# yzqin/s4g-release

Measured on AMD Instinct MI355X. Metric: scenes/sec (25.6k-pt clouds) end-to-end grasp inference, higher is better.
Workload: dtype f32 (f16x2 split)

## Files before the change

include/s4g_ops.h:

```cpp
#ifndef S4G_OPS_H_
#define S4G_OPS_H_

#include <stddef.h>
#include <stdint.h>

#ifdef __cplusplus
extern "C" {
#endif

#define S4G_ABI_VERSION 14


#define S4G_OK 0
#define S4G_EINVAL (-1)
#define S4G_EWORKSPACE (-2)
#define S4G_EUNSUPPORTED (-3)

#define S4G_FLAG_FMAD 1

typedef void *s4g_stream_t;

#define S4G_OP_FPS 1
#define S4G_OP_BALL_QUERY 2
#define S4G_OP_THREE_NN 3
// ... 135 lines not shown
} s4g_gemm_desc_t;

int s4g_mlp_gemm_f32(const s4g_gemm_desc_t *desc, s4g_stream_t stream);

typedef struct s4g_heads_desc {
  int32_t precision, P, N, ldx;
  int32_t C, H0, H1, H2, H3;
  const float *X;
  const void *W_frag[5];
  const float *bias[5];
  const float *w_inv_scale[5];
  float *out[4];
  int32_t channels[4];
  int32_t sigmoid_head;
  const float *a_amax;
  float a_amax_floor;
  int32_t rows_per_scene;
  const void *pre_W_frag[2];
  const float *pre_bias[2];
  const float *pre_w_inv_scale[2];
  const int32_t *pre_nidx;
  const float *pre_nw;
  const float *pre_sparse;
  const float *pre_dense;
  const float *pre_lbias;
  const float *pre_a_amax2;
  int32_t pre_N2;
  int64_t out_batch_stride;
  int32_t head_mask;
} s4g_heads_desc_t;

int s4g_heads_chain_f32(const s4g_heads_desc_t *desc, s4g_stream_t stream);

int s4g_amax_per_scene_f32(const float *x, int64_t B, int64_t n_per_scene, float *out_slots, s4g_stream_t stream);

int s4g_gemm_chain_supported(int loader, int epilogue, int C, int Kpad16);

int s4g_ball_query_i32(const float *xyz_b3n, const float *ctr_b3m, int64_t B,
                       int64_t N, int64_t M, float radius, int64_t K,
                       int32_t *idx_bmk, int32_t *cnt_bm, void *ws,
                       size_t ws_bytes, int flags, s4g_stream_t stream);
int s4g_three_nn_weights_i32(const float *q_b3n1, const float *k_b3n2, int64_t B,
                             int64_t N1, int64_t N2, float eps, int32_t *idx_bn3,
                             float *w_bn3, void *ws, size_t ws_bytes, int flags,
                             s4g_stream_t stream);
size_t s4g_three_nn_grid_workspace_bytes(int64_t B, int64_t N1, int64_t N2);
size_t s4g_three_nn_grid_header_offset(int64_t B, int64_t N2);
int s4g_three_nn_weights_grid_i32(const float *q_b3n1, const float *k_b3n2, int64_t B,
                                  int64_t N1, int64_t N2, float eps, float cell,
                                  int32_t *idx_bn3, float *w_bn3, void *ws,
                                  size_t ws_bytes, int flags, s4g_stream_t stream);

int s4g_three_nn_grid_f32(const float *q_b3n1, const float *k_b3n2, int64_t B, int64_t N1,
                          int64_t N2, float cell, int64_t *idx_bn3, float *d2_bn3, void *ws,
                          size_t ws_bytes, int flags, s4g_stream_t stream);

int s4g_query_group_f32(const float *xyz_b3n, const float *ctr_b3m, int64_t B,
                        int64_t N, int64_t M, float radius, int64_t K,
                        int64_t *idx_bmk, int64_t *cnt_bm, float *grouped_b3mk,
                        void *ws, size_t ws_bytes, int flags, s4g_stream_t stream);

int s4g_group_rel_xyz_i32(const float *xyz_b3n, const float *ctr_b3m, const int32_t *idx_bmk,
                          int64_t B, int64_t N, int64_t M, int64_t K, float *rel_pk4,
                          s4g_stream_t stream);

int s4g_group_rel_xyz_unique_i32(const float *xyz_b3n, const float *ctr_b3m, const int32_t *idx_bmk,
// ... 185 lines not shown
```

s4g_release_amd/_cabi.py:

```python
import ctypes
import os

_HERE = os.path.dirname(os.path.abspath(__file__))
LIB_PATH = os.environ.get("S4G_HIP_LIB") or os.path.join(_HERE, "libs4g_hip.so")

S4G_ABI_VERSION = 14
S4G_EINVAL = -1
S4G_EWORKSPACE = -2
S4G_EUNSUPPORTED = -3
S4G_FLAG_FMAD = 1
S4G_OP_FPS, S4G_OP_BALL_QUERY, S4G_OP_THREE_NN = 1, 2, 3

_vp = ctypes.c_void_p
_i64 = ctypes.c_int64
_sz = ctypes.c_size_t
_int = ctypes.c_int
_f32 = ctypes.c_float

_i32 = ctypes.c_int32


class GemmDesc(ctypes.Structure):
    _fields_ = [
        ("loader", _i32), ("epilogue", _i32), ("groups", _i32), ("relu", _i32),
# ... 3 lines not shown
        ("gidx", _vp), ("feat", _vp), ("xyz", _vp), ("ctr", _vp),
        ("Cf", _i32), ("N", _i32), ("M", _i32), ("K", _i32),
        ("nidx", _vp), ("nw", _vp), ("sparse", _vp), ("dense", _vp),
        ("C2", _i32), ("C1", _i32), ("N2", _i32), ("N1", _i32),
        ("out", _vp), ("ldc", _i32), ("c_coff", _i32), ("c_gcol", _i32),
        ("cf_ptr", _vp * 4), ("cf_start", _i32 * 5), ("cf_sigmoid_from", _i32), ("cf_N", _i32),
        ("precision", _i32), ("Kpad16", _i32), ("W_bf16x3", _vp), ("mlp1_w", _vp),
        ("W_f16x2", _vp), ("w_inv_scale", _vp), ("a_amax", _vp), ("a_amax2", _vp),
        ("a_amax_floor", _f32), ("out_amax", _vp), ("W_f16x2_frag", _vp),
        ("W2_f16x2_frag", _vp), ("w2_inv_scale", _vp), ("bias2", _vp), ("Cout2", _i32), ("relu2", _i32),
        ("W3_f16x2_frag", _vp), ("w3_inv_scale", _vp), ("bias3", _vp), ("Cout3", _i32), ("relu3", _i32),
        ("loader_bias", _vp), ("rows_per_scene", _i32), ("rel_xyz4", _vp), ("seg4", _vp), ("seg_rows", _vp),
        ("out2", _vp), ("ldc2", _i32), ("split_n", _i32), ("out_amax2", _vp),
        ("a_L", _i32),
    ]


class HeadsDesc(ctypes.Structure):
    _fields_ = [
        ("precision", _i32), ("P", _i32), ("N", _i32), ("ldx", _i32),
        ("C", _i32), ("H0", _i32), ("H1", _i32), ("H2", _i32), ("H3", _i32),
        ("X", _vp), ("W_frag", _vp * 5), ("bias", _vp * 5), ("w_inv_scale", _vp * 5),
        ("out", _vp * 4), ("channels", _i32 * 4), ("sigmoid_head", _i32),
        ("a_amax", _vp), ("a_amax_floor", _f32), ("rows_per_scene", _i32),
        ("pre_W_frag", _vp * 2), ("pre_bias", _vp * 2), ("pre_w_inv_scale", _vp * 2),
        ("pre_nidx", _vp), ("pre_nw", _vp), ("pre_sparse", _vp), ("pre_dense", _vp),
        ("pre_lbias", _vp), ("pre_a_amax2", _vp), ("pre_N2", _i32), ("out_batch_stride", _i64), ("head_mask", _i32),
    ]


SIGNATURES = {
    "s4g_mlp_gemm_f32": (_int, [ctypes.POINTER(GemmDesc), _vp]),
    "s4g_heads_chain_f32": (_int, [ctypes.POINTER(HeadsDesc), _vp]),
    "s4g_ball_query_i32": (_int, [_vp, _vp, _i64, _i64, _i64, _f32, _i64, _vp, _vp, _vp, _sz,
                                  _int, _vp]),
    "s4g_three_nn_weights_i32": (_int, [_vp, _vp, _i64, _i64, _i64, _f32, _vp, _vp, _vp, _sz,
                                        _int, _vp]),
    "s4g_three_nn_grid_workspace_bytes": (_sz, [_i64, _i64, _i64]),
    "s4g_three_nn_grid_header_offset": (_sz, [_i64, _i64]),
    "s4g_three_nn_weights_grid_i32": (_int, [_vp, _vp, _i64, _i64, _i64, _f32, _f32, _vp, _vp, _vp,
                                             _sz, _int, _vp]),
    "s4g_three_nn_grid_f32": (_int, [_vp, _vp, _i64, _i64, _i64, _f32, _vp, _vp, _vp, _sz, _int, _vp]),
    "s4g_group_points_xyz_f32": (_int, [_vp, _vp, _i64, _i64, _i64, _i64, _vp, _vp, _sz, _vp]),
    "s4g_gemm_chain_supported": (_int, [_int, _int, _int, _int]),
    "s4g_amax_per_scene_f32": (_int, [_vp, _i64, _i64, _vp, _vp]),
    "s4g_interp_add_cl_f32": (_int, [_vp, _vp, _vp, _vp, _vp, _i64, _i64, _i64, _i64, _int, _vp, _vp, _vp]),
    "s4g_group_points_ws_f32": (_int, [_vp, _vp, _i64, _i64, _i64, _i64, _i64, _vp, _vp, _sz, _vp]),
    "s4g_three_interpolate_ws_f32": (_int, [_vp, _vp, _vp, _i64, _i64, _i64, _i64, _vp, _vp, _sz, _int, _vp]),
    "s4g_fps_gather_i32": (_int, [_vp, _i64, _i64, _i64, _vp, _vp, _vp, _sz, _int, _vp]),
    "s4g_fps_prepass_f32": (_int, [_vp, _i64, _i64, _i64, _vp, _vp, _vp]),
    "s4g_fps_gather_ex_i32": (_int, [_vp, _i64, _i64, _i64, _vp, _vp, _vp, _vp, _vp, _sz, _int, _vp]),
    "s4g_fps_prefix_check_f32": (_int, [_vp, _vp, _i64, _i64, _i64, _vp, _int, _vp]),
    "s4g_build_variants": (_int, []),
    "s4g_test_knobs_enabled": (_int, []),
    "s4g_fps_f64": (_int, [_vp, _i64, _i64, _i64, _vp, _vp, _sz, _int, _vp]),
    "s4g_ball_query_f64": (_int, [_vp, _vp, _i64, _i64, _i64, _f32, _i64, _vp, _vp, _int, _vp]),
    "s4g_three_nn_f64": (_int, [_vp, _vp, _i64, _i64, _i64, _vp, _vp, _int, _vp]),
    "s4g_group_points_f64": (_int, [_vp, _vp, _i64, _i64, _i64, _i64, _i64, _vp, _vp]),
    "s4g_group_points_backward_f64": (_int, [_vp, _vp, _i64, _i64, _i64, _i64, _i64, _vp, _vp]),
    "s4g_three_interpolate_f64": (_int, [_vp, _vp, _vp, _i64, _i64, _i64, _i64, _vp, _int, _vp]),
    "s4g_three_interpolate_backward_f64": (_int, [_vp, _vp, _vp, _i64, _i64, _i64, _i64, _vp, _vp]),
    "s4g_scatter_det_workspace_bytes": (_sz, [_i64, _i64, _i64]),
    "s4g_scatter_det_workspace_bytes_c": (_sz, [_i64, _i64, _i64, _i64, _int]),
    "s4g_group_points_backward_det_f32": (_int, [_vp, _vp, _i64, _i64, _i64, _i64, _i64, _vp, _vp, _sz, _vp]),
    "s4g_three_interpolate_backward_det_f32": (_int, [_vp, _vp, _vp, _i64, _i64, _i64, _i64, _vp, _vp, _sz, _vp]),
    "s4g_group_rel_xyz_i32": (_int, [_vp, _vp, _vp, _i64, _i64, _i64, _i64, _vp, _vp]),
# ... 127 lines not shown
```

s4g_release_amd/csrc/mlp_heads.hip:

```cpp
#include <stdlib.h>

#include "mlp_common.h"

#ifndef S4G_HEADS_ABLATE
#define S4G_HEADS_ABLATE 0
#endif

namespace s4g {

__device__ __forceinline__ void heads_keep_alive(const f32x16& v) { asm volatile("" ::"v"(v)); }

struct HeadsParams {
  int P, N;
  const float* X;
  int ldx;
  const uint16_t* W[5];
  const float* bias[5];
  const float* wsc[5];
  float* out[4];
  int ch[4];
  long long obs[4];
  int head_mask;
  int sigmoid_head;
  const float* a_amax;
  float a_floor;
  int rps;
  const uint16_t* Wp[2];
  const float* bias_p[2];
  const float* wsc_p[2];
  const int* nidx;
  const float* nw;
  const float* sparse;
  const float* dense;
  const float* lbias;
  const float* a_amax2;
  int N2;
};

template <int PL, int HD_RING, int NRBT, bool PRE>
__global__ __launch_bounds__(512, 2) void mlp_heads_kernel(const HeadsParams p) {
  constexpr int BM = 32 * NRBT, C = 256, NW = 8, astr = C + 8, aplane = BM * astr;
  constexpr int FB = PL * 1024;
  extern __shared__ __attribute__((aligned(16))) float smemf[];
  uint16_t* PA = reinterpret_cast<uint16_t*>(smemf);
  uint16_t* PB = PA + PL * aplane;
  float* scr = reinterpret_cast<float*>(PB + PL * aplane);

  const int t = threadIdx.x;
  const int lane = t & 63;
  const int li = lane & 31, lh = lane >> 5;
  const int wv = __builtin_amdgcn_readfirstlane(t >> 6);
  const int p0 = blockIdx.x * BM;
  const uint32_t wf_lane = (uint32_t)lane * 16u;

  float sa = 1.f, inv_sa = 1.f;
  if constexpr (PL == 2) {
    float amax = p.a_floor;
    if constexpr (PRE) {
      if (p.a_amax) amax += amax_rows(p.a_amax, lane, p0, min(p0 + BM, p.P) - 1, p.rps);
      if (p.a_amax2) amax += amax_rows(p.a_amax2, lane, p0, min(p0 + BM, p.P) - 1, p.rps);
    } else if (p.a_amax) {
      amax = fmaxf(amax, amax_rows(p.a_amax, lane, p0, min(p0 + BM, p.P) - 1, p.rps));
    }
    uint32_t ex = __float_as_uint(amax) >> 23;
    ex = ex < 15u ? 15u : (ex > 240u ? 240u : ex);
    ex = __builtin_amdgcn_readfirstlane(ex);
    sa = __uint_as_float((268u - ex) << 23);
    inv_sa = __uint_as_float((ex - 14u) << 23);
  }

  WRef wrs[5];
#pragma unroll
  for (int L = 0; L < 5; ++L) wrs[L] = wref(p.W[L], 0);
  auto woff = [&](int n32, int nks, int ks) { return (size_t)((n32 * nks + ks) * FB); };
  auto w0 = [&](int g, int h) { return wrs[0] + woff(g * 16 + h * 8 + wv, 16, 0); };
  auto w1 = [&](int g, int h) { return wrs[1] + woff(g * 8 + wv, 32, h * 16); };
  auto w2 = [&](int g) { return wrs[2] + woff(g * 8 + wv, 16, 0); };
  auto w3 = [&](int g) { return wrs[3] + woff(g * 4 + (wv & 3), 16, 0); };
  auto wl = [&](int g) { return wrs[4] + woff(g, 8, 0); };
  auto wload = [&](const WRef& w, uint32_t byte_off, int pl) { return wref_load(w, wf_lane + pl * 1024, byte_off); };
  const WRef wp0 = PRE ? wref(p.Wp[0], woff(wv, 16, 0)) : wrs[0];
  const WRef wp1 = PRE ? wref(p.Wp[1], woff(wv, 16, 0)) : wrs[0];

  const int hmask = p.head_mask;
  const int g_first = __builtin_ctz(hmask);
  uint4 ring[HD_RING][PL];
  {
    const WRef w = PRE ? wp0 : w0(g_first, 0);
#pragma unroll
    for (int d = 0; d < HD_RING; ++d)
#pragma unroll
      for (int pl = 0; pl < PL; ++pl) ring[d][pl] = wload(w, d * FB, pl);
  }

#pragma unroll 1
  for (int r0 = 0; r0 < BM; r0 += 64) {
// ... 33 lines not shown
          for (int e = 0; e < 4; ++e) {
            float acc = __fmul_rn(av[e], w3[0]);
            acc = __fadd_rn(acc, __fmul_rn(bv[e], w3[1]));
            acc = __fadd_rn(acc, __fmul_rn(cv[e], w3[2]));
            r[e] = ok ? fmaxf(__fadd_rn(__fadd_rn(yv[e], acc), bi[e]), 0.f) : 0.f;
          }
          ra[h * 4 + kk] = make_float4(r[0], r[1], r[2], r[3]);
        }
      }
    } else {
    const float* src = p.X + (size_t)(ok ? p0 + row : 0) * p.ldx + chunk * 4;
#pragma unroll
    for (int kt = 0; kt < 8; ++kt)
      ra[kt] = ok ? nt_load4(src + kt * 32) : make_float4(0.f, 0.f, 0.f, 0.f);
    }
#pragma unroll
    for (int kt = 0; kt < 8; ++kt) {
      uint16_t* dst = PA + row * astr + kt * 32 + chunk * 4;
      if constexpr (PL == 2) {
        uint2 h, l;
        split2_h<false>(ra[kt], sa, h, l);
        *reinterpret_cast<uint2*>(dst) = h;
        *reinterpret_cast<uint2*>(dst + aplane) = l;
      } else {
        *reinterpret_cast<uint2*>(dst) = make_uint2(cvt_pk_bf16(ra[kt].x, ra[kt].y), cvt_pk_bf16(ra[kt].z, ra[kt].w));
      }
    }
  }
  __syncthreads();

#define S4G_HD_TERM(NRB, PA_, PB_, ZERO)                                                            \
  _Pragma("unroll") for (int rb = 0; rb < NRB; ++rb)                                                \
    acc[rb] = chain_mfma<PL>(bf[PB_], af[rb][PA_], (ZERO) ? zero16 : acc[rb]);
#define S4G_HD_STRIP(PANEL, NRB, ROWOFF, WCUR, NKS, WNEXT)                                          \
  {                                                                                                 \
    const uint16_t* a_lane = (PANEL) + ((ROWOFF) + li) * astr + 8 * lh;                             \
    uint4 afn[NRBT][PL];                                                                            \
    _Pragma("unroll") for (int rb = 0; rb < NRB; ++rb) _Pragma("unroll") for (int pl = 0; pl < PL; ++pl) \
      afn[rb][pl] = *reinterpret_cast<const uint4*>(a_lane + pl * aplane + rb * 32 * astr);         \
    const WRef wcur_ = (WCUR);                                                                      \
    const WRef wnext_ = (WNEXT);                                                                    \
    _Pragma("unroll") for (int ks = 0; ks < NKS; ++ks) {                                            \
      const int d = ks % HD_RING;                                                                   \
      const int ksn = ks + 1 == NKS ? 0 : ks + 1;                                                   \
      uint4 af[NRBT][PL], bf[PL];                                                                   \
      _Pragma("unroll") for (int rb = 0; rb < NRB; ++rb) _Pragma("unroll") for (int pl = 0; pl < PL; ++pl) { \
        af[rb][pl] = afn[rb][pl];                                                                   \
        if (!(S4G_HEADS_ABLATE & 2))                                                                \
          afn[rb][pl] = *reinterpret_cast<const uint4*>(a_lane + pl * aplane + rb * 32 * astr + ksn * 16); \
      }                                                                                             \
      _Pragma("unroll") for (int pl = 0; pl < PL; ++pl) bf[pl] = ring[d][pl];                       \
      {                                                                                             \
        const int kr = ks + HD_RING;                                                                \
        _Pragma("unroll") for (int pl = 0; pl < PL; ++pl)                                           \
          if (!(S4G_HEADS_ABLATE & 1))                                                              \
            ring[d][pl] = kr < NKS ? wload(wcur_, kr * FB, pl) : wload(wnext_, (kr - NKS) * FB, pl); \
      }                                                                                             \
      if constexpr (PL == 2) {                                                                      \
        S4G_HD_TERM(NRB, 0, 1, ks == 0)                                                             \
        S4G_HD_TERM(NRB, 1, 0, false)                                                               \
        S4G_HD_TERM(NRB, 0, 0, false)                                                               \
      } else {                                                                                      \
        S4G_HD_TERM(NRB, 0, 0, ks == 0)                                                             \
      }                                                                                             \
      _Pragma("unroll") for (int q = 0; q < PL; ++q) {                                              \
        __builtin_amdgcn_sched_group_barrier(0x008, 1, 0);                                          \
        __builtin_amdgcn_sched_group_barrier(0x020, 1, 0);                                          \
        __builtin_amdgcn_sched_group_barrier(0x008, 1, 0);                                          \
        __builtin_amdgcn_sched_group_barrier(0x100, 1, 0);                                          \
      }                                                                                             \
      __builtin_amdgcn_sched_barrier(0);                                                            \
    }                                                                                               \
  }

  f32x16 zero16;
#pragma unroll
  for (int r = 0; r < 16; ++r) zero16[r] = 0.f;
  f32x16 acc[NRBT];
  float* epi_s = scr + wv * 64;

  auto stage_sb2 = [&](const float* wsc, const float* bias, int gch, float mul) {
    epi_s[lane] = lane < 32 ? (PL == 2 ? mul * wsc[gch + lane] : 1.f) : bias[gch + lane - 32];
  };
  auto stage_sb = [&](int L, int gch, float mul) { stage_sb2(p.wsc[L], p.bias[L], gch, mul); };

  float inv_sh = 1.f;
  auto panel_epilogue_to = [&](uint16_t* PD, auto nrb_tag, int rowoff, int pch0) {
    constexpr int NRB = decltype(nrb_tag)::value;
    if (S4G_HEADS_ABLATE & 4) {
#pragma unroll
      for (int rb = 0; rb < NRB; ++rb) heads_keep_alive(acc[rb]);
      if (!(S4G_HEADS_ABLATE & 8)) {
        __syncthreads();
        __syncthreads();
      }
      return;
    }
    float tmax = 0.f;
#pragma unroll
    for (int j = 0; j < 4; ++j) {
      const float4 sc4 = *reinterpret_cast<const float4*>(epi_s + 8 * j + 4 * lh);
      const float4 b4 = *reinterpret_cast<const float4*>(epi_s + 32 + 8 * j + 4 * lh);
      const float scv[4] = {sc4.x, sc4.y, sc4.z, sc4.w};
      const float bv[4] = {b4.x, b4.y, b4.z, b4.w};
#pragma unroll
      for (int rb = 0; rb < NRB; ++rb) {
        const f32x2 x01 = pk_fma(f32x2{acc[rb][4 * j], acc[rb][4 * j + 1]}, f32x2{scv[0], scv[1]}, f32x2{bv[0], bv[1]});
        const f32x2 x23 = pk_fma(f32x2{acc[rb][4 * j + 2], acc[rb][4 * j + 3]}, f32x2{scv[2], scv[3]}, f32x2{bv[2], bv[3]});
        const float x[4] = {fmaxf(x01.x, 0.f), fmaxf(x01.y, 0.f), fmaxf(x23.x, 0.f), fmaxf(x23.y, 0.f)};
#pragma unroll
        for (int e = 0; e < 4; ++e) acc[rb][4 * j + e] = x[e];
        if constexpr (PL == 2) {
          tmax = fmaxf(fmaxf(tmax, x[0]), x[1]);
          tmax = fmaxf(fmaxf(tmax, x[2]), x[3]);
        }
      }
    }
    float sh = 1.f;
    if constexpr (PL == 2) {
      const uint32_t wm = wave_max_u32(__float_as_uint(tmax));
      if (lane == 0) scr[NW * 64 + wv] = __uint_as_float(wm);
    }
    __syncthreads();
    if constexpr (PL == 2) {
      float hmax = scr[NW * 64];
#pragma unroll
      for (int w = 1; w < NW; ++w) hmax = fmaxf(hmax, scr[NW * 64 + w]);
      uint32_t exh = __float_as_uint(hmax) >> 23;
      exh = exh < 15u ? 15u : (exh > 240u ? 240u : exh);
      exh = __builtin_amdgcn_readfirstlane(exh);
      sh = __uint_as_float((268u - exh) << 23);
      inv_sh = __uint_as_float((exh - 14u) << 23);
    }
#pragma unroll
    for (int j = 0; j < 4; ++j)
#pragma unroll
      for (int rb = 0; rb < NRB; ++rb) {
        uint16_t* dst = PD + (rowoff + rb * 32 + li) * astr + pch0 + 8 * j + 4 * lh;
        if constexpr (PL == 2) {
          const float4 v = make_float4(acc[rb][4 * j], acc[rb][4 * j + 1], acc[rb][4 * j + 2], acc[rb][4 * j + 3]);
          uint2 h, l;
          split2_h<false>(v, sh, h, l);
          *reinterpret_cast<uint2*>(dst) = h;
          *reinterpret_cast<uint2*>(dst + aplane) = l;
        } else {
          *reinterpret_cast<uint2*>(dst) = make_uint2(cvt_pk_bf16(acc[rb][4 * j], acc[rb][4 * j + 1]),
                                                      cvt_pk_bf16(acc[rb][4 * j + 2], acc[rb][4 * j + 3]));
        }
      }
    __syncthreads();
  };
  auto panel_epilogue = [&](auto nrb_tag, int rowoff, int pch0) { panel_epilogue_to(PB, nrb_tag, rowoff, pch0); };
  using full = std::integral_constant<int, NRBT>;
  using half = std::integral_constant<int, NRBT / 2>;

  if constexpr (PRE) {
    stage_sb2(p.wsc_p[0], p.bias_p[0], wv * 32, inv_sa);
    S4G_HD_STRIP(PA, NRBT, 0, wp0, 16, wp1)
    panel_epilogue(full{}, 0, wv * 32);
    stage_sb2(p.wsc_p[1], p.bias_p[1], wv * 32, inv_sh);
    S4G_HD_STRIP(PB, NRBT, 0, wp1, 16, w0(g_first, 0))
    panel_epilogue_to(PA, full{}, 0, wv * 32);
    inv_sa = inv_sh;
  }

  for (int g = g_first, gn; g >= 0; g = gn) {
    const int rest = hmask >> (g + 1);
    gn = rest ? g + 1 + __builtin_ctz(rest) : -1;
    const int gnx = gn >= 0 ? gn : g;
    f32x16 acc1[NRBT];
    stage_sb(0, g * 512 + wv * 32, inv_sa);
    S4G_HD_STRIP(PA, NRBT, 0, w0(g, 0), 16, w1(g, 0))
    panel_epilogue(full{}, 0, wv * 32);
    S4G_HD_STRIP(PB, NRBT, 0, w1(g, 0), 16, w0(g, 1))
#pragma unroll
    for (int rb = 0; rb < NRBT; ++rb)
#pragma unroll
      for (int r = 0; r < 16; r += 2) {
        const f32x2 v = f32x2{acc[rb][r], acc[rb][r + 1]} * f32x2{inv_sh, inv_sh};
        acc1[rb][r] = v.x;
        acc1[rb][r + 1] = v.y;
      }
    stage_sb(0, g * 512 + 256 + wv * 32, inv_sa);
    S4G_HD_STRIP(PA, NRBT, 0, w0(g, 1), 16, w1(g, 1))
    panel_epilogue(full{}, 0, wv * 32);
    S4G_HD_STRIP(PB, NRBT, 0, w1(g, 1), 16, w2(g))
#pragma unroll
    for (int rb = 0; rb < NRBT; ++rb)
#pragma unroll
      for (int r = 0; r < 16; r += 2) {
        const f32x2 v = pk_fma(f32x2{acc[rb][r], acc[rb][r + 1]}, f32x2{inv_sh, inv_sh}, f32x2{acc1[rb][r], acc1[rb][r + 1]});
        acc[rb][r] = v.x;
        acc[rb][r + 1] = v.y;
      }
    stage_sb(1, g * 256 + wv * 32, 1.f);
    panel_epilogue(full{}, 0, wv * 32);
    stage_sb(2, g * 256 + wv * 32, inv_sh);
    S4G_HD_STRIP(PB, NRBT, 0, w2(g), 16, w3(g))
    panel_epilogue(full{}, 0, wv * 32);
    {
      const int row3 = (wv >> 2) * (BM / 2), cg = wv & 3;
      stage_sb(3, g * 128 + cg * 32, inv_sh);
      const WRef after = wv < NRBT ? wl(g) : w0(gnx, 0);
      S4G_HD_STRIP(PB, NRBT / 2, row3, w3(g), 16, after)
      panel_epilogue(half{}, row3, cg * 32);
    }
    if (wv < NRBT) {
      stage_sb(4, g * 32, inv_sh);
      S4G_HD_STRIP(PB, 1, wv * 32, wl(g), 8, w0(gnx, 0))
      const int row = p0 + wv * 32 + li;
      const int b = row / p.N, pt = row - b * p.N;
      const int nch = p.ch[g];
      float* __restrict__ base = p.out[g] + (size_t)b * (size_t)p.obs[g] + pt;
#pragma unroll
      for (int j = 0; j < 4; ++j) {
        const float4 sc4 = *reinterpret_cast<const float4*>(epi_s + 8 * j + 4 * lh);
        const float4 b4 = *reinterpret_cast<const float4*>(epi_s + 32 + 8 * j + 4 * lh);
        const float scv[4] = {sc4.x, sc4.y, sc4.z, sc4.w};
        const float bv[4] = {b4.x, b4.y, b4.z, b4.w};
#pragma unroll
        for (int e = 0; e < 4; ++e) {
          const int c = 8 * j + 4 * lh + e;
          float x = __fmaf_rn(acc[0][4 * j + e], scv[e], bv[e]);
          if (g == p.sigmoid_head) x = 1.0f / (1.0f + expf(-x));
          if (c < nch && row < p.P) base[(size_t)c * p.N] = x;
        }
      }
    }
  }
#undef S4G_HD_STRIP
#undef S4G_HD_TERM
}

template <int PL, int HD_RING, int NRBT, bool PRE>
static int launch_heads_cfg(const HeadsParams& p, hipStream_t st) {
  constexpr int BM = 32 * NRBT;
  constexpr size_t lds = sizeof(uint16_t) * 2 * PL * BM * (256 + 8) + sizeof(float) * (8 * 64 + 16);
  static_assert(lds <= 160 * 1024, "one workgroup's panels must fit a CU's LDS");
  static LdsAttrCache lds_cache;
  if (int rc = allow_dynamic_lds(reinterpret_cast<const void*>(&mlp_heads_kernel<PL, HD_RING, NRBT, PRE>), lds, lds_cache)) return rc;
  hipLaunchKernelGGL((mlp_heads_kernel<PL, HD_RING, NRBT, PRE>), dim3((unsigned)((p.P + BM - 1) / BM)), dim3(512), lds, st, p);
  S4G_LAUNCH_CHECK();
  return S4G_OK;
}
template <int PL, int HD_RING, int NRBT>
static int launch_heads(const HeadsParams& p, hipStream_t st) {
  return p.Wp[0] ? launch_heads_cfg<PL, HD_RING, NRBT, true>(p, st) : launch_heads_cfg<PL, HD_RING, NRBT, false>(p, st);
}

}

extern "C" int s4g_heads_chain_f32(const s4g_heads_desc_t* d, s4g_stream_t stream) {
  using namespace s4g;
  if (!d || d->P < 0 || d->N <= 0) return S4G_EINVAL;
  const bool pre = d->pre_W_frag[0] != nullptr;
  if (!pre && (!d->X || (d->ldx & 3) || d->ldx < 256 || ((uintptr_t)d->X & 15))) return S4G_EINVAL;
  if (pre && (!d->pre_W_frag[1] || !d->pre_bias[0] || !d->pre_bias[1] || !d->pre_nidx || !d->pre_nw ||
              !d->pre_sparse || !d->pre_lbias || d->pre_N2 < 3 || ((uintptr_t)d->pre_sparse & 15) ||
              ((uintptr_t)d->pre_dense & 15) || ((uintptr_t)d->pre_lbias & 15) ||
              (d->precision == S4G_GEMM_F16X2 && (!d->pre_w_inv_scale[0] || !d->pre_w_inv_scale[1]))))
    return S4G_EINVAL;
  if (d->precision != S4G_GEMM_F16X2 && d->precision != S4G_GEMM_BF16) return S4G_EINVAL;
  if (d->C != 256 || d->H0 != 512 || d->H1 != 256 || d->H2 != 256 || d->H3 != 128) return S4G_EUNSUPPORTED;
  HeadsParams p;
  p.P = d->P;
  p.N = d->N;
  p.X = d->X;
  p.ldx = d->ldx;
  for (int l = 0; l < 5; ++l) {
    if (!d->W_frag[l] || !d->bias[l] || (d->precision == S4G_GEMM_F16X2 && !d->w_inv_scale[l])) return S4G_EINVAL;
    p.W[l] = (const uint16_t*)d->W_frag[l];
    p.bias[l] = d->bias[l];
    p.wsc[l] = d->w_inv_scale[l];
  }
  p.head_mask = d->head_mask ? d->head_mask : 15;
  if (p.head_mask < 0 || p.head_mask > 15) return S4G_EINVAL;
  for (int h = 0; h < 4; ++h) {
    p.out[h] = nullptr;
    p.ch[h] = 0;
    p.obs[h] = 0;
    if (!((p.head_mask >> h) & 1)) continue;
    if (!d->out[h] || d->channels[h] <= 0 || d->channels[h] > 32) return S4G_EINVAL;
    p.out[h] = d->out[h];
    p.ch[h] = d->channels[h];
    if (d->out_batch_stride != 0 && d->out_batch_stride < (int64_t)d->channels[h] * d->N) return S4G_EINVAL;
    p.obs[h] = d->out_batch_stride != 0 ? (long long)d->out_batch_stride : (long long)d->channels[h] * d->N;
  }
  p.sigmoid_head = d->sigmoid_head;
  p.a_amax = d->a_amax;
  p.a_floor = d->a_amax_floor;
  p.rps = d->rows_per_scene > 0 ? d->rows_per_scene : 0;
  for (int l = 0; l < 2; ++l) {
    p.Wp[l] = pre ? (const uint16_t*)d->pre_W_frag[l] : nullptr;
    p.bias_p[l] = pre ? d->pre_bias[l] : nullptr;
    p.wsc_p[l] = pre ? d->pre_w_inv_scale[l] : nullptr;
  }
  p.nidx = pre ? d->pre_nidx : nullptr;
  p.nw = pre ? d->pre_nw : nullptr;
  p.sparse = pre ? d->pre_sparse : nullptr;
  p.dense = pre ? d->pre_dense : nullptr;
  p.lbias = pre ? d->pre_lbias : nullptr;
  p.a_amax2 = pre ? d->pre_a_amax2 : nullptr;
  p.N2 = pre ? d->pre_N2 : 0;
  if (d->precision == S4G_GEMM_F16X2 && !d->a_amax && !(d->a_amax_floor > 0.f)) return S4G_EINVAL;
  if (d->P == 0) return S4G_OK;
  hipStream_t st = (hipStream_t)stream;
  if (d->precision == S4G_GEMM_F16X2) return launch_heads<2, 4, 2>(p, st);
  return launch_heads<1, 4, 4>(p, st);
}
```

s4g_release_amd/fused.py:

```python
import ctypes
import os

import torch

from . import _cabi
from . import functions as _F

_i32 = ctypes.c_int32
_fp = ctypes.c_void_p
GemmDesc = _cabi.GemmDesc
HeadsDesc = _cabi.HeadsDesc

LOAD_PLAIN, LOAD_GATHER, LOAD_INTERP, LOAD_GATHER_MLP1, LOAD_GATHER_ADD, LOAD_INTERP_ADD = 0, 1, 2, 3, 4, 5
EPI_STORE, EPI_MAX, EPI_CF = 0, 1, 2

NETWORK_KINDS = {(9, 4): "PN2_CLS", (6, 3): "PN2"}
HEADS_CLS = ("score", "frame_R", "frame_t", "movable_logits")
HEADS_CONTACT = ("scene_score_logits", "frame_R", "frame_t", "movable_logits")
CONTACT_RAW_CHANNELS = (3, 6, 3, 5)
CONTACT_OUT_CHANNELS = (3, 9, 3, 5)


def fold_conv_bn(block):
    w = block.conv.weight.detach().double().flatten(1)
# ... 35 lines not shown
    ex = torch.where(amax > 0, ex, torch.zeros_like(ex)).clamp(-100, 100)
    one = torch.ones_like(amax)
    s = torch.ldexp(one, 15 - ex)
    ws = w * s[..., None]
    w1 = ws.to(torch.float16)
    w2 = (ws - w1.float()).to(torch.float16)
    return torch.stack([w1, w2], dim=0).contiguous(), torch.ldexp(one, ex - 15).contiguous()


def fragment_order(planes):
    if planes.dim() == 3:
        planes = planes.unsqueeze(1)
    npl, G, cout, k16 = planes.shape
    x = planes.reshape(npl, G, cout // 32, 32, k16 // 16, 2, 8)
    return x.permute(1, 2, 4, 0, 5, 3, 6).contiguous()


class _Layer:

    def __init__(self, W, bias, cin, groups=1):
        self.W = W.contiguous()
        self.bias = bias.contiguous()
        self.groups = groups
        self.cout = self.W.shape[-2]
        self.kpad = self.W.shape[-1]
        self.cin = cin
        self.kpad16 = (self.kpad + 15) // 16 * 16
        w16 = self.W.new_zeros(self.W.shape[:-1] + (self.kpad16,))
        w16[..., :self.kpad] = self.W
        self.W3 = split_bf16x3(w16)
        self.Wh2, self.w_inv_scale = split_f16x2(w16)
        self.Wfrag = fragment_order(self.Wh2) if self.cout % 32 == 0 else None
        self.Wfrag_bf16 = fragment_order(self.W3[:1])[:, :, :, 0].contiguous() if self.cout % 32 == 0 else None


_STREAM_POOL = {}


def _stream_pool(dev, n_geo, n_dense):
    key = (str(dev), int(n_geo), int(n_dense))
    pool = _STREAM_POOL.get(key)
    if pool is None:
        pool = _STREAM_POOL[key] = ([torch.cuda.Stream(device=dev, priority=-1) for _ in range(n_geo)],
                                    [torch.cuda.Stream(device=dev) for _ in range(n_dense)])
    return pool


class FusedPointNet2:

    def __init__(self, net, precision=None, fold_only=False, check_finite=False):
        self.check_finite = bool(check_finite)
        if precision is None:
            precision = os.environ.get("S4G_GEMM_MODE", "f16x2")
        if precision not in ("f16x2", "bf16x3", "fp32", "bf16"):
            raise ValueError("precision must be 'f16x2', 'bf16x3', 'fp32' or 'bf16'")
        self.precision = precision
        self.dense_streams = max(1, int(os.environ.get("S4G_DENSE_STREAMS", "1")))
        self.fuse2 = _cabi.knob("S4G_GEMM_FUSE2", "1") != "0"
        self.fp_linear_first = _cabi.knob("S4G_FP_LINEAR_FIRST", "1") != "0"
        self.geo_streams = max(1, int(os.environ.get("S4G_GEO_STREAMS", "2")))
        self.rel_xyz = _cabi.knob("S4G_REL_XYZ", "1") != "0"
        self.sa_unique = _cabi.knob("S4G_SA_UNIQUE", "1") != "0"
        self.heads_pre = _cabi.knob("S4G_HEADS_PRE", "1") != "0"
        self.merge_shared = _cabi.knob("S4G_MERGE_SHARED", "1") != "0"
        self.fp_chain_next = _cabi.knob("S4G_FP_CHAIN_NEXT", "1") != "0"
        self.fps_prefix = _cabi.knob("S4G_FPS_PREFIX", "1") != "0"
# ... 68 lines not shown
        b0 = torch.cat([f[0][1] for f in folded], dim=0)
        self.head_layers.append(_Layer(_pad_k(w0), b0, w0.shape[1]))
        for li in range(1, depth):
            W = torch.stack([_pad_k(f[li][0]) for f in folded], dim=0)
            bias = torch.stack([f[li][1] for f in folded], dim=0)
            self.head_layers.append(_Layer(W, bias, folded[0][li][0].shape[1], groups=4))
        chans = [lg.weight.shape[0] for _, lg in heads]
        self.head_channels = chans
        cl = heads[0][1].weight.shape[1]
        wl = torch.zeros((sum(chans), 4 * cl), dtype=torch.float32, device=self.dev)
        bl = torch.zeros((sum(chans),), dtype=torch.float32, device=self.dev)
        r = 0
        for h, (_, lg) in enumerate(heads):
            c = lg.weight.shape[0]
            wl[r:r + c, h * cl:(h + 1) * cl] = lg.weight.detach().flatten(1)
            bl[r:r + c] = lg.bias.detach()
            r += c
        self.logit_layer = _Layer(_pad_k(wl), bl, 4 * cl)
        self.sigmoid_from = sum(chans[:3])
        self._streams = None
        hl = self.head_layers
        self.heads_fused = None
        if (precision in ("f16x2", "bf16") and depth == 4 and
                hl[0].cin == 256 and hl[0].cout == 4 * 512 and
                [(l.cout, l.cin, l.groups) for l in hl[1:]] == [(256, 512, 4), (256, 256, 4), (128, 256, 4)] and
                cl == 128 and max(chans) <= 32 and len(chans) == 4):
            wpad = torch.zeros((4, 32, cl), dtype=torch.float32, device=self.dev)
            bpad = torch.zeros((4, 32), dtype=torch.float32, device=self.dev)
            for h, (_, lg) in enumerate(heads):
                c = lg.weight.shape[0]
                wpad[h, :c] = lg.weight.detach().flatten(1)
                bpad[h, :c] = lg.bias.detach()
            self.heads_fused = list(hl) + [_Layer(wpad, bpad, cl, groups=4)]

    def packed_weights(self):
        out = {}

        def put(prefix, layer):
            for a in ("W", "bias", "W3", "Wh2", "w_inv_scale", "Wfrag", "Wfrag_bf16"):
                t = getattr(layer, a)
                if t is not None:
                    out["%s.%s" % (prefix, a)] = t
        for li, sa in enumerate(self.sa):
            for l, layer in enumerate(sa["layers"]):
                put("sa%d.%d" % (li, l), layer)
            if sa["mlp1"] is not None:
                out["sa%d.mlp1" % li] = sa["mlp1"]
            if sa["pre"] is not None:
                put("sa%d.pre" % li, sa["pre"]["la"])
                out["sa%d.pre.w1" % li] = sa["pre"]["w1"]
            out["sa%d.meta" % li] = torch.tensor([sa["M"], sa["K"], sa["cf"], sa["radius"], sa["mlp1_bound"],
                                                  0.0 if sa["pre"] is None else sa["pre"]["bound"]],
                                                 dtype=torch.float64)
        for fi, fp in enumerate(self.fp):
            for l, layer in enumerate(fp["layers"]):
                put("fp%d.%d" % (fi, l), layer)
            out["fp%d.meta" % fi] = torch.tensor([fp["eps"], fp["bias0_max"]], dtype=torch.float64)
        for l, layer in enumerate(self.head_layers):
            put("heads.%d" % l, layer)
        put("heads.logits", self.logit_layer)
        if self.heads_fused is not None:
            put("heads.logits_padded", self.heads_fused[-1])
        return out

    def _fusable(self, l1, l2, loader=LOAD_PLAIN, epi=EPI_STORE):
        c = l1.cout
# ... 699 lines not shown
```

Baseline: 2055.

## Use precomputed weight-norm bounds to pick f16x2 split scales in heads epilogue

```diff
diff --git a/include/s4g_ops.h b/include/s4g_ops.h
--- a/include/s4g_ops.h
+++ b/include/s4g_ops.h
@@ -191,6 +191,9 @@
 
 int s4g_heads_chain_f32(const s4g_heads_desc_t *desc, s4g_stream_t stream);
 
+int s4g_panel_bounds_set(const void *w_frag, int groups, const float *n, const float *bm);
+int s4g_panel_bounds_drop(const void *w_frag);
+
 int s4g_amax_per_scene_f32(const float *x, int64_t B, int64_t n_per_scene, float *out_slots, s4g_stream_t stream);
 
 int s4g_gemm_chain_supported(int loader, int epilogue, int C, int Kpad16);
diff --git a/s4g_release_amd/_cabi.py b/s4g_release_amd/_cabi.py
--- a/s4g_release_amd/_cabi.py
+++ b/s4g_release_amd/_cabi.py
@@ -59,6 +59,8 @@
 SIGNATURES = {
     "s4g_mlp_gemm_f32": (_int, [ctypes.POINTER(GemmDesc), _vp]),
     "s4g_heads_chain_f32": (_int, [ctypes.POINTER(HeadsDesc), _vp]),
+    "s4g_panel_bounds_set": (_int, [_vp, _int, ctypes.POINTER(ctypes.c_float), ctypes.POINTER(ctypes.c_float)]),
+    "s4g_panel_bounds_drop": (_int, [_vp]),
     "s4g_ball_query_i32": (_int, [_vp, _vp, _i64, _i64, _i64, _f32, _i64, _vp, _vp, _vp, _sz,
                                   _int, _vp]),
     "s4g_three_nn_weights_i32": (_int, [_vp, _vp, _i64, _i64, _i64, _f32, _vp, _vp, _vp, _sz,
diff --git a/s4g_release_amd/csrc/mlp_heads.hip b/s4g_release_amd/csrc/mlp_heads.hip
--- a/s4g_release_amd/csrc/mlp_heads.hip
+++ b/s4g_release_amd/csrc/mlp_heads.hip
@@ -1,4 +1,8 @@
 #include <stdlib.h>
+
+#include <mutex>
+#include <unordered_map>
+#include <vector>
 
 #include "mlp_common.h"
 
@@ -7,6 +11,11 @@
 #endif
 
 namespace s4g {
+
+#ifdef S4G_CHAIN_STAMPS
+__device__ unsigned long long g_heads_stamps[512 * 8];
+#define S4G_HD_NOW() __builtin_amdgcn_s_memtime()
+#endif
 
 __device__ __forceinline__ void heads_keep_alive(const f32x16& v) { asm volatile("" ::"v"(v)); }
 
@@ -35,10 +44,13 @@
   const float* lbias;
   const float* a_amax2;
   int N2;
+  float bnd_n[4][4], bnd_b[4][4];
+  float bnd_np[2], bnd_bp[2];
 };
 
-template <int PL, int HD_RING, int NRBT, bool PRE>
+template <int PL, int HD_RING, int NRBT, bool PRE, bool BND>
 __global__ __launch_bounds__(512, 2) void mlp_heads_kernel(const HeadsParams p) {
+  static_assert(!BND || PL == 2, "bounds scale the f16x2 panels only");
   constexpr int BM = 32 * NRBT, C = 256, NW = 8, astr = C + 8, aplane = BM * astr;
   constexpr int FB = PL * 1024;
   extern __shared__ __attribute__((aligned(16))) float smemf[];
@@ -54,6 +66,7 @@
   const uint32_t wf_lane = (uint32_t)lane * 16u;
 
   float sa = 1.f, inv_sa = 1.f;
+  float in_max_a = 0.f;
   if constexpr (PL == 2) {
     float amax = p.a_floor;
     if constexpr (PRE) {
@@ -62,6 +75,7 @@
     } else if (p.a_amax) {
       amax = fmaxf(amax, amax_rows(p.a_amax, lane, p0, min(p0 + BM, p.P) - 1, p.rps));
     }
+    in_max_a = amax;
     uint32_t ex = __float_as_uint(amax) >> 23;
     ex = ex < 15u ? 15u : (ex > 240u ? 240u : ex);
     ex = __builtin_amdgcn_readfirstlane(ex);
@@ -161,7 +175,7 @@
 #define S4G_HD_TERM(NRB, PA_, PB_, ZERO)                                                            \
   _Pragma("unroll") for (int rb = 0; rb < NRB; ++rb)                                                \
     acc[rb] = chain_mfma<PL>(bf[PB_], af[rb][PA_], (ZERO) ? zero16 : acc[rb]);
-#define S4G_HD_STRIP(PANEL, NRB, ROWOFF, WCUR, NKS, WNEXT)                                          \
+#define S4G_HD_STRIP(PANEL, NRB, ROWOFF, WCUR, NKS, WNEXT, FENCE)                                   \
   {                                                                                                 \
     const uint16_t* a_lane = (PANEL) + ((ROWOFF) + li) * astr + 8 * lh;                             \
     uint4 afn[NRBT][PL];                                                                            \
@@ -173,6 +187,7 @@
       const int d = ks % HD_RING;                                                                   \
       const int ksn = ks + 1 == NKS ? 0 : ks + 1;                                                   \
       uint4 af[NRBT][PL], bf[PL];                                                                   \
+      if (BND && (FENCE) && ks == NKS - 1) __syncthreads();    \
       _Pragma("unroll") for (int rb = 0; rb < NRB; ++rb) _Pragma("unroll") for (int pl = 0; pl < PL; ++pl) { \
         af[rb][pl] = afn[rb][pl];                                                                   \
         if (!(S4G_HEADS_ABLATE & 2))                                                                \
@@ -214,8 +229,67 @@
   auto stage_sb = [&](int L, int gch, float mul) { stage_sb2(p.wsc[L], p.bias[L], gch, mul); };
 
   float inv_sh = 1.f;
+  float sh_o = 1.f, inv_o = 1.f, in_max_b = 0.f;
+  int par = 0;
+  auto set_bound = [&](float n, float bm, float in_max) {
+    uint32_t exb = __float_as_uint(__fmaf_rn(n, in_max, bm)) >> 23;
+    exb = exb < 15u ? 15u : (exb > 240u ? 240u : exb);
+    exb = __builtin_amdgcn_readfirstlane(exb);
+    sh_o = __uint_as_float((268u - exb) << 23);
+    inv_o = __uint_as_float((exb - 14u) << 23);
+  };
+#ifdef S4G_CHAIN_STAMPS
+  const int stamp_b = (int)blockIdx.x - max(0, ((int)gridDim.x - 512) / 2);
+  const bool stamp_on = wv == 0 && stamp_b >= 0 && stamp_b < 512;
+  unsigned long long st_acc[5] = {0, 0, 0, 0, 0};
+  const unsigned long long st_begin = S4G_HD_NOW();
+#endif
   auto panel_epilogue_to = [&](uint16_t* PD, auto nrb_tag, int rowoff, int pch0) {
     constexpr int NRB = decltype(nrb_tag)::value;
+#ifdef S4G_CHAIN_STAMPS
+    const unsigned long long st0 = S4G_HD_NOW();
+    unsigned long long st1 = st0, st2 = st0;
+#endif
+    if constexpr (BND) {
+      float tmax = 0.f;
+#pragma unroll
+      for (int j = 0; j < 4; ++j) {
+        const float4 sc4 = *reinterpret_cast<const float4*>(epi_s + 8 * j + 4 * lh);
+        const float4 b4 = *reinterpret_cast<const float4*>(epi_s + 32 + 8 * j + 4 * lh);
+#pragma unroll
+        for (int rb = 0; rb < NRB; ++rb) {
+          const f32x2 x01 = pk_fma(f32x2{acc[rb][4 * j], acc[rb][4 * j + 1]}, f32x2{sc4.x, sc4.y}, f32x2{b4.x, b4.y});
+          const f32x2 x23 = pk_fma(f32x2{acc[rb][4 * j + 2], acc[rb][4 * j + 3]}, f32x2{sc4.z, sc4.w}, f32x2{b4.z, b4.w});
+          const float4 v = make_float4(fmaxf(x01.x, 0.f), fmaxf(x01.y, 0.f), fmaxf(x23.x, 0.f), fmaxf(x23.y, 0.f));
+          tmax = fmaxf(fmaxf(tmax, v.x), v.y);
+          tmax = fmaxf(fmaxf(tmax, v.z), v.w);
+          uint16_t* dst = PD + (rowoff + rb * 32 + li) * astr + pch0 + 8 * j + 4 * lh;
+          uint2 h, l;
+          split2_h<false>(v, sh_o, h, l);
+#ifdef S4G_CHAIN_STAMPS
+          if (j == 0 && rb == 0) st1 = S4G_HD_NOW();
+#endif
+          *reinterpret_cast<uint2*>(dst) = h;
+          *reinterpret_cast<uint2*>(dst + aplane) = l;
+        }
+      }
+#ifdef S4G_CHAIN_STAMPS
+      st2 = S4G_HD_NOW();
+#endif
+      const uint32_t wm = wave_max_u32(__float_as_uint(tmax));
+      if (lane == 0) scr[NW * 64 + par * NW + wv] = __uint_as_float(wm);
+      __syncthreads();
+      const float4 m0 = *reinterpret_cast<const float4*>(scr + NW * 64 + par * NW);
+      const float4 m1 = *reinterpret_cast<const float4*>(scr + NW * 64 + par * NW + 4);
+      in_max_b = fmaxf(fmaxf(fmaxf(m0.x, m0.y), fmaxf(m0.z, m0.w)), fmaxf(fmaxf(m1.x, m1.y), fmaxf(m1.z, m1.w)));
+      par ^= 1;
+      inv_sh = inv_o;
+#ifdef S4G_CHAIN_STAMPS
+      const unsigned long long st3 = S4G_HD_NOW();
+      st_acc[0] += st1 - st0, st_acc[1] += st2 - st0, st_acc[2] += st3 - st0, st_acc[3] += 1;
+#endif
+      return;
+    }
     if (S4G_HEADS_ABLATE & 4) {
 #pragma unroll
       for (int rb = 0; rb < NRB; ++rb) heads_keep_alive(acc[rb]);
@@ -246,6 +320,9 @@
       }
     }
     float sh = 1.f;
+#ifdef S4G_CHAIN_STAMPS
+    const unsigned long long st_r = S4G_HD_NOW();
+#endif
     if constexpr (PL == 2) {
       const uint32_t wm = wave_max_u32(__float_as_uint(tmax));
       if (lane == 0) scr[NW * 64 + wv] = __uint_as_float(wm);
@@ -270,6 +347,9 @@
           const float4 v = make_float4(acc[rb][4 * j], acc[rb][4 * j + 1], acc[rb][4 * j + 2], acc[rb][4 * j + 3]);
           uint2 h, l;
           split2_h<false>(v, sh, h, l);
+#ifdef S4G_CHAIN_STAMPS
+          if (j == 0 && rb == 0) st1 = S4G_HD_NOW();
+#endif
           *reinterpret_cast<uint2*>(dst) = h;
           *reinterpret_cast<uint2*>(dst + aplane) = l;
         } else {
@@ -277,7 +357,14 @@
                                                       cvt_pk_bf16(acc[rb][4 * j + 2], acc[rb][4 * j + 3]));
         }
       }
+#ifdef S4G_CHAIN_STAMPS
+    st2 = S4G_HD_NOW();
+#endif
     __syncthreads();
+#ifdef S4G_CHAIN_STAMPS
+    const unsigned long long st3 = S4G_HD_NOW();
+    st_acc[0] += st1 - st0, st_acc[1] += st2 - st0, st_acc[2] += st3 - st0, st_acc[3] += 1, st_acc[4] += st_r - st0;
+#endif
   };
   auto panel_epilogue = [&](auto nrb_tag, int rowoff, int pch0) { panel_epilogue_to(PB, nrb_tag, rowoff, pch0); };
   using full = std::integral_constant<int, NRBT>;
@@ -285,12 +372,15 @@
 
   if constexpr (PRE) {
     stage_sb2(p.wsc_p[0], p.bias_p[0], wv * 32, inv_sa);
-    S4G_HD_STRIP(PA, NRBT, 0, wp0, 16, wp1)
+    if constexpr (BND) set_bound(p.bnd_np[0], p.bnd_bp[0], in_max_a);
+    S4G_HD_STRIP(PA, NRBT, 0, wp0, 16, wp1, true)
     panel_epilogue(full{}, 0, wv * 32);
     stage_sb2(p.wsc_p[1], p.bias_p[1], wv * 32, inv_sh);
-    S4G_HD_STRIP(PB, NRBT, 0, wp1, 16, w0(g_first, 0))
+    if constexpr (BND) set_bound(p.bnd_np[1], p.bnd_bp[1], in_max_b);
+    S4G_HD_STRIP(PB, NRBT, 0, wp1, 16, w0(g_first, 0), false)
     panel_epilogue_to(PA, full{}, 0, wv * 32);
     inv_sa = inv_sh;
+    in_max_a = in_max_b;
   }
 
   for (int g = g_first, gn; g >= 0; g = gn) {
@@ -299,9 +389,11 @@
     const int gnx = gn >= 0 ? gn : g;
     f32x16 acc1[NRBT];
     stage_sb(0, g * 512 + wv * 32, inv_sa);
-    S4G_HD_STRIP(PA, NRBT, 0, w0(g, 0), 16, w1(g, 0))
+    if constexpr (BND) set_bound(p.bnd_n[0][g], p.bnd_b[0][g], in_max_a);
+    S4G_HD_STRIP(PA, NRBT, 0, w0(g, 0), 16, w1(g, 0), true)
     panel_epilogue(full{}, 0, wv * 32);
-    S4G_HD_STRIP(PB, NRBT, 0, w1(g, 0), 16, w0(g, 1))
+    const float in_max_h0 = in_max_b;
+    S4G_HD_STRIP(PB, NRBT, 0, w1(g, 0), 16, w0(g, 1), false)
 #pragma unroll
     for (int rb = 0; rb < NRBT; ++rb)
 #pragma unroll
@@ -311,9 +403,10 @@
         acc1[rb][r + 1] = v.y;
       }
     stage_sb(0, g * 512 + 256 + wv * 32, inv_sa);
-    S4G_HD_STRIP(PA, NRBT, 0, w0(g, 1), 16, w1(g, 1))
+    S4G_HD_STRIP(PA, NRBT, 0, w0(g, 1), 16, w1(g, 1), true)
     panel_epilogue(full{}, 0, wv * 32);
-    S4G_HD_STRIP(PB, NRBT, 0, w1(g, 1), 16, w2(g))
+    if constexpr (BND) set_bound(p.bnd_n[1][g], p.bnd_b[1][g], fmaxf(in_max_h0, in_max_b));
+    S4G_HD_STRIP(PB, NRBT, 0, w1(g, 1), 16, w2(g), true)
 #pragma unroll
     for (int rb = 0; rb < NRBT; ++rb)
 #pragma unroll
@@ -325,18 +418,20 @@
     stage_sb(1, g * 256 + wv * 32, 1.f);
     panel_epilogue(full{}, 0, wv * 32);
     stage_sb(2, g * 256 + wv * 32, inv_sh);
-    S4G_HD_STRIP(PB, NRBT, 0, w2(g), 16, w3(g))
+    if constexpr (BND) set_bound(p.bnd_n[2][g], p.bnd_b[2][g], in_max_b);
+    S4G_HD_STRIP(PB, NRBT, 0, w2(g), 16, w3(g), true)
     panel_epilogue(full{}, 0, wv * 32);
     {
       const int row3 = (wv >> 2) * (BM / 2), cg = wv & 3;
       stage_sb(3, g * 128 + cg * 32, inv_sh);
+      if constexpr (BND) set_bound(p.bnd_n[3][g], p.bnd_b[3][g], in_max_b);
       const WRef after = wv < NRBT ? wl(g) : w0(gnx, 0);
-      S4G_HD_STRIP(PB, NRBT / 2, row3, w3(g), 16, after)
+      S4G_HD_STRIP(PB, NRBT / 2, row3, w3(g), 16, after, true)
       panel_epilogue(half{}, row3, cg * 32);
     }
     if (wv < NRBT) {
       stage_sb(4, g * 32, inv_sh);
-      S4G_HD_STRIP(PB, 1, wv * 32, wl(g), 8, w0(gnx, 0))
+      S4G_HD_STRIP(PB, 1, wv * 32, wl(g), 8, w0(gnx, 0), false)
       const int row = p0 + wv * 32 + li;
       const int b = row / p.N, pt = row - b * p.N;
       const int nch = p.ch[g];
@@ -359,22 +454,43 @@
   }
 #undef S4G_HD_STRIP
 #undef S4G_HD_TERM
-}
-
-template <int PL, int HD_RING, int NRBT, bool PRE>
+#ifdef S4G_CHAIN_STAMPS
+  if (stamp_on && lane == 0) {
+    for (int i = 0; i < 5; ++i) g_heads_stamps[stamp_b * 8 + i] = st_acc[i];
+    g_heads_stamps[stamp_b * 8 + 5] = S4G_HD_NOW() - st_begin;
+  }
+#endif
+}
+
+template <int PL, int HD_RING, int NRBT, bool PRE, bool BND>
 static int launch_heads_cfg(const HeadsParams& p, hipStream_t st) {
   constexpr int BM = 32 * NRBT;
   constexpr size_t lds = sizeof(uint16_t) * 2 * PL * BM * (256 + 8) + sizeof(float) * (8 * 64 + 16);
   static_assert(lds <= 160 * 1024, "one workgroup's panels must fit a CU's LDS");
   static LdsAttrCache lds_cache;
-  if (int rc = allow_dynamic_lds(reinterpret_cast<const void*>(&mlp_heads_kernel<PL, HD_RING, NRBT, PRE>), lds, lds_cache)) return rc;
-  hipLaunchKernelGGL((mlp_heads_kernel<PL, HD_RING, NRBT, PRE>), dim3((unsigned)((p.P + BM - 1) / BM)), dim3(512), lds, st, p);
+  if (int rc = allow_dynamic_lds(reinterpret_cast<const void*>(&mlp_heads_kernel<PL, HD_RING, NRBT, PRE, BND>), lds, lds_cache)) return rc;
+  hipLaunchKernelGGL((mlp_heads_kernel<PL, HD_RING, NRBT, PRE, BND>), dim3((unsigned)((p.P + BM - 1) / BM)), dim3(512), lds, st, p);
   S4G_LAUNCH_CHECK();
   return S4G_OK;
 }
-template <int PL, int HD_RING, int NRBT>
+template <int PL, int HD_RING, int NRBT, bool BND>
 static int launch_heads(const HeadsParams& p, hipStream_t st) {
-  return p.Wp[0] ? launch_heads_cfg<PL, HD_RING, NRBT, true>(p, st) : launch_heads_cfg<PL, HD_RING, NRBT, false>(p, st);
+  return p.Wp[0] ? launch_heads_cfg<PL, HD_RING, NRBT, true, BND>(p, st)
+                 : launch_heads_cfg<PL, HD_RING, NRBT, false, BND>(p, st);
+}
+
+static std::mutex g_bounds_mu;
+static std::unordered_map<const void*, std::vector<float>> g_bounds;
+
+bool panel_bounds_lookup(const void* w_frag, int groups, float* n, float* bm) {
+  std::lock_guard<std::mutex> lk(g_bounds_mu);
+  const auto it = g_bounds.find(w_frag);
+  if (it == g_bounds.end() || (int)it->second.size() != 2 * groups) return false;
+  for (int g = 0; g < groups; ++g) {
+    n[g] = it->second[2 * g];
+    bm[g] = it->second[2 * g + 1];
+  }
+  return true;
 }
 
 }
@@ -431,9 +547,41 @@
   p.lbias = pre ? d->pre_lbias : nullptr;
   p.a_amax2 = pre ? d->pre_a_amax2 : nullptr;
   p.N2 = pre ? d->pre_N2 : 0;
+  for (int l = 0; l < 4; ++l)
+    for (int g = 0; g < 4; ++g) p.bnd_n[l][g] = p.bnd_b[l][g] = 0.f;
+  p.bnd_np[0] = p.bnd_np[1] = p.bnd_bp[0] = p.bnd_bp[1] = 0.f;
   if (d->precision == S4G_GEMM_F16X2 && !d->a_amax && !(d->a_amax_floor > 0.f)) return S4G_EINVAL;
   if (d->P == 0) return S4G_OK;
   hipStream_t st = (hipStream_t)stream;
-  if (d->precision == S4G_GEMM_F16X2) return launch_heads<2, 4, 2>(p, st);
-  return launch_heads<1, 4, 4>(p, st);
-}
+  if (d->precision == S4G_GEMM_F16X2) {
+    bool bnd = true;
+    for (int l = 0; l < 4 && bnd; ++l) bnd = panel_bounds_lookup(d->W_frag[l], 4, p.bnd_n[l], p.bnd_b[l]);
+    for (int l = 0; l < 2 && bnd && pre; ++l) bnd = panel_bounds_lookup(d->pre_W_frag[l], 1, &p.bnd_np[l], &p.bnd_bp[l]);
+    return bnd ? launch_heads<2, 4, 2, true>(p, st) : launch_heads<2, 4, 2, false>(p, st);
+  }
+  return launch_heads<1, 4, 4, false>(p, st);
+}
+
+extern "C" int s4g_panel_bounds_set(const void* w_frag, int groups, const float* n, const float* bm) {
+  if (!w_frag || groups < 1 || groups > 64 || !n || !bm) return S4G_EINVAL;
+  std::vector<float> v((size_t)2 * groups);
+  for (int g = 0; g < groups; ++g) {
+    if (!(n[g] >= 0.f) || !(bm[g] >= 0.f) || !(n[g] <= 3.0e38f) || !(bm[g] <= 3.0e38f)) return S4G_EINVAL;
+    v[2 * g] = n[g];
+    v[2 * g + 1] = bm[g];
+  }
+  std::lock_guard<std::mutex> lk(s4g::g_bounds_mu);
+  s4g::g_bounds[w_frag] = std::move(v);
+  return S4G_OK;
+}
+
+extern "C" int s4g_panel_bounds_drop(const void* w_frag) {
+  std::lock_guard<std::mutex> lk(s4g::g_bounds_mu);
+  return (int)s4g::g_bounds.erase(w_frag);
+}
+
+#ifdef S4G_CHAIN_STAMPS
+extern "C" int s4g_debug_heads_stamps(unsigned long long* host_out_512x8) {
+  return (int)hipMemcpyFromSymbol(host_out_512x8, HIP_SYMBOL(s4g::g_heads_stamps), sizeof(unsigned long long) * 512 * 8);
+}
+#endif
diff --git a/s4g_release_amd/fused.py b/s4g_release_amd/fused.py
--- a/s4g_release_amd/fused.py
+++ b/s4g_release_amd/fused.py
@@ -91,6 +91,42 @@
         self.Wh2, self.w_inv_scale = split_f16x2(w16)
         self.Wfrag = fragment_order(self.Wh2) if self.cout % 32 == 0 else None
         self.Wfrag_bf16 = fragment_order(self.W3[:1])[:, :, :, 0].contiguous() if self.cout % 32 == 0 else None
+
+
+PANEL_BOUND_MARGIN = 1.0 + 2.0 ** -13
+
+
+def _f32_up(x):
+    import numpy as np
+    x = np.asarray(x, dtype=np.float64)
+    y = x.astype(np.float32)
+    return np.where(y.astype(np.float64) < x, np.nextafter(y, np.float32(np.inf)), y).astype(np.float32)
+
+
+def panel_bounds(layer, groups=None):
+    groups = layer.groups if groups is None else groups
+    W = layer.W.detach().double().cpu().reshape(groups, -1, layer.W.shape[-1])
+    b = layer.bias.detach().double().cpu().reshape(groups, -1)
+    n = W.abs().sum(dim=-1).amax(dim=-1).numpy() * PANEL_BOUND_MARGIN
+    bm = b.abs().amax(dim=-1).numpy() * PANEL_BOUND_MARGIN
+    return _f32_up(n), _f32_up(bm)
+
+
+def register_panel_bounds(layer, groups=None, scale_n=1.0):
+    import weakref
+    fl = ctypes.POINTER(ctypes.c_float)
+    n, bm = panel_bounds(layer, groups)
+    n = (n * scale_n).astype("float32")
+    ptr = layer.Wfrag.data_ptr()
+    _cabi.check(_cabi.lib().s4g_panel_bounds_set(ptr, len(n), n.ctypes.data_as(fl), bm.ctypes.data_as(fl)),
+                "panel_bounds_set")
+    weakref.finalize(layer.Wfrag, drop_panel_bounds, ptr)
+    return n, bm
+
+
+def drop_panel_bounds(ptr):
+    if _cabi._lib is not None:
+        _cabi._lib.s4g_panel_bounds_drop(ptr)
 
 
 _STREAM_POOL = {}
@@ -225,6 +261,12 @@
                 wpad[h, :c] = lg.weight.detach().flatten(1)
                 bpad[h, :c] = lg.bias.detach()
             self.heads_fused = list(hl) + [_Layer(wpad, bpad, cl, groups=4)]
+            if precision == "f16x2" and not fold_only:
+                for layer in self.heads_fused[:4]:
+                    register_panel_bounds(layer, groups=4)
+                for layer in (self.fp[-1]["layers"][1:] if self.fp else ()):
+                    if layer.Wfrag is not None and layer.groups == 1:
+                        register_panel_bounds(layer)
 
     def packed_weights(self):
         out = {}
```

Result: no change. 2054 (-0.1%).
